# dmalyuta/explicit_hybrid_mpc

Hardware: AMD Instinct MI355X
Metric: oracle LP solves/sec + final regions/sec, 4-state 2-input N=5 hybrid MPC (higher is better)
Workload: dtype f64

## Files before the change

explicit_hybrid_mpc_amd/_capi.py:

```python

import ctypes
import os
import numpy as np

from . import build as _build

c_double_p = ctypes.POINTER(ctypes.c_double)
c_int32_p = ctypes.POINTER(ctypes.c_int32)
c_uint8_p = ctypes.POINTER(ctypes.c_uint8)

EHM_OK = 0
EHM_E_INVALID = -1
EHM_E_NO_DEVICE = -2
EHM_E_HIP = -3
EHM_E_CAPACITY = -4
EHM_E_INFEASIBLE = -5
EHM_E_NUMERIC = -6
PERSIST_FAMILIES = ('none', 'k2', 'kp', 'kpm', 'k4')
EHM_MAX_P = 8

EXPORTED = [
    'ehm_problem_create', 'ehm_problem_destroy', 'ehm_problem_set_eps', 'ehm_sync',
    'ehm_stream', 'ehm_solve_ptd_batch', 'ehm_feas_ptd_batch', 'ehm_solve_pt_batch',
    'ehm_vr_batch', 'ehm_slack_batch', 'ehm_bar_e_batch', 'ehm_min_simplex_batch',
# ... 64 lines not shown


class NodeInit(ctypes.Structure):
    _fields_ = [('delta', c_uint8_p), ('vcost', c_double_p), ('vinput', c_double_p)]


class TreeInfo(ctypes.Structure):
    _fields_ = [('n_nodes', ctypes.c_int64), ('n_leaves', ctypes.c_int64),
                ('n_roots', ctypes.c_int64), ('n_closed', ctypes.c_int64),
                ('lp_solves', ctypes.c_int64), ('ref_solves', ctypes.c_int64),
                ('ipm_iters', ctypes.c_int64), ('sweeps', ctypes.c_int64),
                ('max_depth', ctypes.c_int32), ('truncated', ctypes.c_int32),
                ('volume_closed', ctypes.c_double), ('min_margin', ctypes.c_double),
                ('device_seconds', ctypes.c_double), ('decide_seconds', ctypes.c_double),
                ('expand_seconds', ctypes.c_double), ('decide_launches', ctypes.c_int64),
                ('expand_launches', ctypes.c_int64), ('decide_solves', ctypes.c_int64),
                ('decide_iters', ctypes.c_int64), ('replicated_closed', ctypes.c_int64),
                ('replicated_nodes', ctypes.c_int64), ('replicated_solves', ctypes.c_int64),
                ('cert_closed', ctypes.c_int64), ('witness_open', ctypes.c_int64),
                ('swaps', ctypes.c_int64), ('blacklisted', ctypes.c_int64),
                ('kind_solves', ctypes.c_int64 * 5), ('kind_iters', ctypes.c_int64 * 5),
                ('near_threshold', ctypes.c_int64), ('witness_inherited', ctypes.c_int64),
                ('midpoints_shared', ctypes.c_int64),
                ('persist_ticks', ctypes.c_int64 * 10), ('witness_table', ctypes.c_int64)]


class Progress(ctypes.Structure):
    _fields_ = [('n_nodes', ctypes.c_int64), ('n_closed', ctypes.c_int64),
                ('frontier', ctypes.c_int64), ('sweeps', ctypes.c_int64),
                ('lp_solves', ctypes.c_int64), ('ipm_iters', ctypes.c_int64),
                ('depth', ctypes.c_int32), ('reserved', ctypes.c_int32),
                ('volume_closed', ctypes.c_double), ('n_splits', ctypes.c_int64)]


class PwaLaw(ctypes.Structure):
    _fields_ = [('n_x', ctypes.c_int32), ('n_u', ctypes.c_int32), ('n_modes', ctypes.c_int32),
                ('N', ctypes.c_int32), ('A', c_double_p), ('B', c_double_p), ('w', c_double_p),
                ('region_rows', c_int32_p), ('Hx', c_double_p), ('hx', c_double_p),
                ('n_gx', ctypes.c_int32), ('Gx', c_double_p), ('gx', c_double_p),
                ('n_gu', ctypes.c_int32), ('Gu', c_double_p), ('gu', c_double_p),
                ('n_q', ctypes.c_int32), ('Q', c_double_p),
                ('n_r', ctypes.c_int32), ('R', c_double_p)]


POINTS_FN = ctypes.CFUNCTYPE(ctypes.c_int, ctypes.c_void_p, ctypes.c_int64, ctypes.c_void_p,
                             ctypes.c_void_p, ctypes.c_int32, ctypes.c_int32, ctypes.c_void_p,
                             ctypes.c_void_p)
# ... 235 lines not shown
```

explicit_hybrid_mpc_amd/csrc/ehm_capi.hip:

```cpp
#include <hip/hip_runtime.h>

#include <algorithm>
#include <cmath>
#include <cstdarg>
#include <cstdio>
#include <cstdlib>
#include <cstring>
#include <memory>
#include <set>
#include <string>
#include <vector>

#include "../../include/ehmpc.h"
#include "ehm_host.h"

#define EHM_MAX_P_DEV 8
#include "ehm_kernels.h"
#include "ehm_k2.h"
#include "ehm_implicit.h"

using namespace ehm;

#define EHM_K2_NPS(X, S) X(8, S) X(12, S) X(16, S) X(20, S) X(24, S) X(28, S) X(32, S)
#define EHM_K2_ALL(X) EHM_K2_NPS(X, 1) EHM_K2_NPS(X, 2) EHM_K2_NPS(X, 3) EHM_K2_NPS(X, 4)
// ... 403 lines not shown
    DevBuf rec, left, didx, depth, flags, tstar, grad, wit, mt_state, mt_data;
};

struct ehm_problem {
    int device = 0;
    Stream stream;
    DevProblem dp{};
    int delta_len = 0;
    std::vector<uint8_t> deltas;
    DevBuf consts;
    DevBuf wc2;
    DevBuf wc4;
    DevBuf wr3;
    DevBuf quad;
    bool quadratic = false;
    bool k2q_ok = false;
    bool v1_ok = false;
    int decide_full = 0;
    int mid_first = 1;
    int inherit_wit = 1;
    bool budget_keep = false;
    bool check_witness = false;
    int work_first = 1;
    int share_mid = 1;
    int any_admissible = 0;
    int hy_timing = 0;
    int solver_gen = 2;
    DevBuf seg;
    std::set<const K2Api*> k2_ready;
    std::set<const KpApi*> kp_ready;
    NodePool pool_cache;
    DevBuf fr_a, fr_b, open_flag, open_list, d_count;
    DevBuf pq_slots, pq_ctl;
    DevBuf in0, in1, in2, out0, out1, out2, out3;
    DevBuf ex_stage, ex_tmp;
    DevBuf d_cnt;
    DevCounters* counters() const { return d_cnt.as<DevCounters>(); }
    struct ehm_tree* active_run = nullptr;
    std::vector<struct ehm_tree*> trees;
    Event bev[2];
    double batch_seconds[2] = {0.0, 0.0};
    long long batch_launches[2] = {0, 0};
    long long launches = 0;
    long long fallbacks = 0;
    long long slivers = 0;
    int num_cu = 256;
// ... 6 lines not shown
    ehm_problem* prob = nullptr;
    int device = 0;
    std::unique_ptr<HyState> hy;
    DevTree dt{};
    NodePool pool;
    long long limit = 0;
    DevBuf code;
    ehm_tree_info info{};
    int skip_volume = 0;
    int32_t persist_kernel[4] = {0, 0, 0, 0};
    bool unordered = false;
    bool keep_ids = false;
    DevBuf d_perm, d_inv;
    bool have_perm = false;
    struct Run {
        bool active = false;
        int max_depth = 0, action = 0, shard_world = 1, shard_rank = 0, engine = 0;
        int deal_depth = 0;
        long long shard_min = 0;
        bool sharded = true, cur_is_a = true;
        long long n_roots = 0, n_nodes = 0, nf = 0, n_closed = 0, ref_solves = 0;
        long long pre_closed = 0, pre_nodes = 0, pre_solves = 0, given = 0, received = 0;
        long long pre_first = 0;
        int sweeps = 0, depth = 0, truncated = 0;
        DevCounters c0{};
        Event ev0;
        std::vector<Event> evs;
        std::vector<int> ev_kind;
    } run;
    ~ehm_tree();
};

static int map_deltas(ehm_problem* P, int64_t n_inst, const uint8_t* delta,
                      std::vector<int32_t>& out) {
    out.resize((size_t)n_inst);
    const int L = P->delta_len;
    for (int64_t k = 0; k < n_inst; ++k) {
        int found = -1;
        if (!delta) {
            found = 0;
        } else {
            for (int d = 0; d < P->dp.n_delta; ++d) {
                bool eq = true;
                for (int q = 0; q < L && eq; ++q)
                    eq = ((delta[k * L + q] != 0) == (P->deltas[(size_t)d * L + q] != 0));
                if (eq) {
// ... 510 lines not shown
    if (!strcmp(name, "solver")) return ehm_problem_set_solver(P, (int)value);
    if (!strcmp(name, "decide_full")) {
        P->decide_full = value != 0.0;
        return EHM_OK;
    }
    if (!strcmp(name, "timing")) {
        P->hy_timing = value != 0.0;
        return EHM_OK;
    }
    if (!strcmp(name, "mid_first")) {
        P->mid_first = value != 0.0;
        return EHM_OK;
    }
    if (!strcmp(name, "inherit_witness")) {
        P->inherit_wit = value != 0.0;
        return EHM_OK;
    }
    if (!strcmp(name, "work_first")) {
        P->work_first = value != 0.0;
        return EHM_OK;
    }
    if (!strcmp(name, "check_witness")) {
        P->check_witness = value != 0.0;
        return EHM_OK;
    }
    if (!strcmp(name, "budget_keep")) {
        P->budget_keep = value != 0.0;
        return EHM_OK;
    }
    if (!strcmp(name, "share_midpoints")) {
        P->share_mid = value != 0.0;
        return EHM_OK;
    }
    if (!strcmp(name, "any_admissible")) {
        if (value < 0.0 || value > 2e9) return fail(EHM_E_INVALID, "any_admissible: seed + 1, or 0");
        if (P->active_run)
            return fail(EHM_E_INVALID, "any_admissible: not while a partition run is active");
        P->any_admissible = (int)value;
        return EHM_OK;
    }
    return fail(EHM_E_INVALID, "unknown option '%s'", name);
}

int ehm_sync(ehm_problem* P) {
    if (!P) return fail(EHM_E_INVALID, "null problem");
    HIP_TRY(hipStreamSynchronize(P->stream), EHM_E_HIP);
// ... 1302 lines not shown
                }
                const size_t lds = (shared + (size_t)nw * wave) * sizeof(double);
                const long long reg_wg = (kp->max_threads / 64) / nw;
                const long long wg_per_cu =
                    std::max<long long>(1, std::min<long long>(EHM_LDS_BUDGET / lds, reg_wg));
                cfg.L.grid = (int)((long long)P->num_cu * wg_per_cu);
                cfg.L.threads = (int)(64 * nw);
                cfg.L.lds_bytes = lds;
                cfg.L.wave_doubles = (int)wave;
            }
        }
    }
    const long long waves = (long long)cfg.L.grid * (cfg.L.threads / 64);
    const long long n_slots = 2 * T->limit + waves + 64;
    if (n_slots > 0x7fffffffLL || T->limit >= (long long)EHM_REQUEUED)
        return fail(EHM_E_INVALID, "node pool too large for the persistent engine");
    HIP_TRY(P->pq_slots.ensure((size_t)n_slots * 4), EHM_E_HIP);
    HIP_TRY(P->pq_ctl.ensure(sizeof(PersistCtl)), EHM_E_HIP);
    int32_t* slots = P->pq_slots.as<int32_t>();
    HIP_TRY(hipMemsetAsync(slots, 0xFF, (size_t)n_slots * 4, P->stream), EHM_E_HIP);
    const int32_t* cur = (R.cur_is_a ? P->fr_a : P->fr_b).as<int32_t>();
    HIP_TRY(hipMemcpyAsync(slots, cur, (size_t)R.nf * 4, hipMemcpyDeviceToDevice, P->stream),
            EHM_E_HIP);
    PersistDeal deal{0, 0, 0, 1, 0, 0};
    deal.check = P->check_witness ? 1 : 0;
    T->dt.code = nullptr;
    if (dealt) {
        deal = PersistDeal{0, R.deal_depth, R.shard_rank, R.shard_world,
                           getenv("EHM_DEAL_LOW_BITS") ? 0 : 1, 0, P->check_witness ? 1 : 0};
        HIP_TRY(T->code.ensure((size_t)T->pool.cap * 4), EHM_E_HIP);
        T->dt.code = T->code.as<uint32_t>();
        std::vector<uint32_t> codes((size_t)R.n_roots);
        for (long long k = 0; k < R.n_roots; ++k) codes[(size_t)k] = (uint32_t)k;
        HIP_TRY(hipMemcpyAsync(T->dt.code, codes.data(), codes.size() * 4, hipMemcpyHostToDevice,
                               P->stream), EHM_E_HIP);
        HIP_TRY(hipStreamSynchronize(P->stream), EHM_E_HIP);
    }
    if (max_pops > 0 && max_pops < n_slots) deal.pop_limit = (int)max_pops;
    deal.keep = (P->work_first && !getenv("EHM_NO_WORKFIRST")) ? 1 : 0;
    if (deal.pop_limit > 0 && !P->budget_keep) deal.keep = 0;
    PersistCtl h{};
    h.head = 0;
    h.tail = (int)R.nf;
    h.pending = (int)R.nf;
    h.n_nodes = (int)R.n_nodes;
    HIP_TRY(hipMemcpyAsync(P->pq_ctl.ptr, &h, sizeof h, hipMemcpyHostToDevice, P->stream),
            EHM_E_HIP);
    R.evs.push_back(Event::recorded(P->stream));
    if (kp) {
        T->persist_kernel[0] = kp_mid ? EHM_PERSIST_KPM : EHM_PERSIST_KP;
        T->persist_kernel[1] = kp->np_decide;
        T->persist_kernel[2] = kp->np_expand;
        T->persist_kernel[3] = kp->slots;
    } else {
        T->persist_kernel[0] = cfg.api == ehm_k4_api() ? EHM_PERSIST_K4 : EHM_PERSIST_K2;
        T->persist_kernel[1] = cfg.api->np;
        T->persist_kernel[2] = cfg.api->np;
        T->persist_kernel[3] = cfg.api->slots;
    }
    (kp ? kp->persist : cfg.api->persist)(cfg.L, P->dp, T->dt, slots, (int)n_slots,
                                          P->pq_ctl.as<PersistCtl>(), (int)T->limit, P->counters(),
                                          P->decide_full ? 0 : 1, R.max_depth, deal);
    R.evs.push_back(Event::recorded(P->stream));
    R.ev_kind.push_back(0);
    P->launches++;
    HIP_TRY(hipGetLastError(), EHM_E_HIP);
    HIP_TRY(hipMemcpyAsync(&h, P->pq_ctl.ptr, sizeof h, hipMemcpyDeviceToHost, P->stream),
            EHM_E_HIP);
    HIP_TRY(hipStreamSynchronize(P->stream), EHM_E_HIP);
    if (h.abort == 1)
        return fail(EHM_E_CAPACITY, "node pool exhausted at %d nodes (max_nodes=%lld)",
                    h.n_nodes, T->limit);
    const long long left_over =
        (deal.pop_limit > 0 && h.tail > deal.pop_limit) ? (long long)h.tail - deal.pop_limit : 0;
    if (h.abort != 0 || h.pending != left_over)
        return fail(EHM_E_HIP, "persistent frontier kernel stopped early (abort=%d, pending=%d, "
                               "expected %lld)", h.abort, h.pending, left_over);
    if (left_over > 0) {
        DevBuf& fb = P->fr_a;
        HIP_TRY(fb.ensure((size_t)left_over * 4 * 2), EHM_E_HIP);
        HIP_TRY(hipMemcpyAsync(fb.ptr, slots + deal.pop_limit, (size_t)left_over * 4,
                               hipMemcpyDeviceToDevice, P->stream), EHM_E_HIP);
        HIP_TRY(hipStreamSynchronize(P->stream), EHM_E_HIP);
        R.cur_is_a = true;
    }
    R.ref_solves += (long long)h.closed + 3LL * (long long)h.splits;
    if (deal.world > 1) {
        R.pre_closed = (long long)h.repl_closed;
        R.pre_nodes = R.n_roots + 2LL * (long long)h.repl_splits;
        R.pre_solves = (long long)h.repl_solves;
        R.sharded = true;
    }
    R.n_closed += (long long)h.closed;
    R.n_nodes = h.n_nodes;
    R.truncated = R.truncated || h.truncated;
    R.depth = std::max(R.depth, h.max_depth_seen);
    R.sweeps = R.depth + 1;
    R.nf = left_over;
    T->unordered = true;
    return EHM_OK;
}

int ehm_partition_advance(ehm_tree* T, int64_t max_pops, int64_t* frontier_size) {
    if (!T || !T->run.active) return fail(EHM_E_INVALID, "no partition run in progress");
    ehm_problem* P = T->prob;
    auto& R = T->run;
    if (T->hy || P->solver_gen != 2 || P->dp.Wr3)
        return fail(EHM_E_INVALID, "ehm_partition_advance: needs a single-commutation problem on "
                                   "the shared-block kernels (use ehm_partition_step)");
// ... 337 lines not shown
    T->info.n_nodes = R.n_nodes;
    T->info.n_roots = R.n_roots;
    T->info.n_leaves = R.n_nodes - (R.n_nodes - R.n_roots - received) / 2;
    T->info.n_closed = R.n_closed;
    T->info.lp_solves = (int64_t)(c1.lp_solves - R.c0.lp_solves);
    T->info.ipm_iters = (int64_t)(c1.ipm_iters - R.c0.ipm_iters);
    T->info.ref_solves = R.ref_solves;
    T->info.sweeps = R.sweeps;
    T->info.max_depth = R.depth;
    T->info.truncated = R.truncated;
    T->info.device_seconds = ms * 1e-3;
    T->info.decide_seconds = t_kind[0];
    T->info.expand_seconds = t_kind[1];
    T->info.decide_launches = n_kind[0];
    T->info.expand_launches = n_kind[1];
    T->info.decide_solves = (int64_t)(c1.slack_solves - R.c0.slack_solves);
    T->info.decide_iters = (int64_t)(c1.slack_iters - R.c0.slack_iters);
    T->info.cert_closed = (int64_t)(c1.cert_closed - R.c0.cert_closed);
    T->info.witness_open = (int64_t)(c1.wit_open - R.c0.wit_open);
    T->info.witness_inherited = (int64_t)(c1.wit_inherited - R.c0.wit_inherited);
    T->info.midpoints_shared = (int64_t)(c1.mid_shared - R.c0.mid_shared);
    T->info.witness_table = (int64_t)(c1.wit_table - R.c0.wit_table);
    for (int k = 0; k < 10; ++k) T->info.persist_ticks[k] = (int64_t)(c1.prof[k] - R.c0.prof[k]);
    T->info.near_threshold = (int64_t)(c1.routed - R.c0.routed);
    T->info.replicated_closed = R.pre_closed;
    T->info.replicated_nodes = R.pre_nodes;
    T->info.replicated_solves = R.pre_solves;
    {
        double mm;
        std::memcpy(&mm, &c1.min_margin_bits, 8);
        T->info.min_margin = mm;
    }
    for (int k = 0; k < 5; ++k) T->info.kind_solves[k] = T->info.kind_iters[k] = 0;
    T->info.kind_solves[LP_SLACK] = T->info.decide_solves;
    T->info.kind_iters[LP_SLACK] = T->info.decide_iters;
    T->info.kind_solves[LP_POINT] = T->info.lp_solves - T->info.decide_solves;
    T->info.kind_iters[LP_POINT] = T->info.ipm_iters - T->info.decide_iters;
    T->info.swaps = 0;
    T->info.blacklisted = 0;
    if (T->hy) {
        rc = hy_kind_totals(T, T->info.kind_solves, T->info.kind_iters);
        if (rc) return rc;
        T->info.decide_solves = T->info.kind_solves[LP_MIN_SIMPLEX] + T->info.kind_solves[LP_SLACK] +
                                T->info.kind_solves[LP_FEAS_SIMPLEX];
        T->info.decide_iters = T->info.kind_iters[LP_MIN_SIMPLEX] + T->info.kind_iters[LP_SLACK] +
                               T->info.kind_iters[LP_FEAS_SIMPLEX];
// ... 152 lines not shown
```

explicit_hybrid_mpc_amd/csrc/ehm_k2.h:

```cpp
#pragma once

#include <hip/hip_runtime.h>
#include <stdint.h>

#include "ehm_dev.h"

#ifndef EHM_K2_THREADS
#define EHM_K2_THREADS 768
#endif

#define K2_AUG_MIN 32
#define K2_HOT_GRAD 176
#define EHM_ROUTE_TOL 1e-6
#define EHM_REQUEUED 0x40000000

namespace ehm {

__host__ __device__ inline size_t k2_node_doubles(int p, int n_u) {
    const size_t nrec = ((size_t)rec_doubles(p, n_u) + 7) & ~(size_t)7;
    const size_t aug = (2 * (size_t)p * p > K2_AUG_MIN) ? 2 * (size_t)p * p : K2_AUG_MIN;
    return (nrec + aug + (size_t)p * p + 8 + 1) & ~(size_t)1;
}

__host__ __device__ inline int k2_stash_doubles(int p, int n_u) {
// ... 5 lines not shown
    const int r = m & 63;
    return (r != 0 && r + ne <= 64) ? m : ((m + 63) & ~63);
}
__host__ __device__ inline int lp_slots(int m, int ne) {
    return (lp_xbase(m, ne) + ne + 63) >> 6;
}

struct PersistCtl {
    int head;
    int pad0[31];
    int tail;
    int pad1[31];
    int pending;
    int pad2[31];
    int n_nodes;
    int pad3[31];
    int abort;
    int max_depth_seen;
    int truncated;
    int pad4;
    unsigned long long closed;
    unsigned long long splits;
    unsigned long long repl_closed, repl_splits, repl_solves;
};

struct PersistDeal {
    int pop_limit;
    int depth, rank, world;
    int mix;
    int keep;
    int check;
};

struct K2Gather {
    const long long* src;
    const int32_t* dst;
    const int32_t* n_dev;
    int v_off;
    double* grad;
    int sign_mode;
    MidTable pt;
};

struct K2Launch {
    int grid;
    int threads;
    size_t lds_bytes;
    int wave_doubles;
    hipStream_t stream;
    int wc_lds;
};

struct K2Api {
    int np, slots, max_threads, threads_per_lp;
// ... 34 lines not shown
```

explicit_hybrid_mpc_amd/csrc/ehm_persist.h:

```cpp
#ifndef EHM_PERSIST_H
#define EHM_PERSIST_H

#ifndef kx_persist
#error "kx_persist (the kernel's name) must be defined, and the namespace aliases kd / ke declared"
#endif

#define EHM_PERSIST_WATCHDOG_TICKS (60LL * 100000000LL)
#ifndef EHM_PERSIST_MIDFIRST
#define EHM_PERSIST_MIDFIRST 0
#endif
__global__ __launch_bounds__(EHM_K2_THREADS) void kx_persist(
    DevProblem P, DevTree T, int32_t* slots, int n_slots, PersistCtl* ctl, int node_cap,
    DevCounters* cnt, int wave_doubles, int sign_only, int max_depth, PersistDeal deal) {
    double* sm = reinterpret_cast<double*>(k2_smem);
    const int tid = threadIdx.x;
    const int lane0 = tid & 63;
    const int wave = __builtin_amdgcn_readfirstlane(tid >> 6);
    kd::Shared S;
    kd::carve_shared(S, sm, P);
    ke::Shared Se;
    ke::carve_shared(Se, sm, P);
#if EHM2_PROF
    S.gprof = cnt ? cnt->phase : nullptr;
    Se.gprof = cnt ? cnt->phase : nullptr;
#endif
    kd::NodeBuf nb;
    kd::carve_node(nb, sm + kd::shared_doubles(P) + (size_t)wave * wave_doubles, P.p, P.n_u);
    ke::NodeBuf nbe;
    ke::carve_node(nbe, sm + kd::shared_doubles(P) + (size_t)wave * wave_doubles, P.p, P.n_u);
    const int p = P.p, n_u = P.n_u;
    const int nrec = rec_doubles(p, n_u);
    kd::load_shared(P, 0, sm, tid, blockDim.x);
    __syncthreads();
    const long long t_start = wall_clock64();
    unsigned long long* wst = reinterpret_cast<unsigned long long*>(nb.aug);
    double* wmargin = nb.aug + 16;
    enum { W_SOLVES = 0, W_ITERS, W_STALLED, W_ERRORS, W_SLACK, W_SLACK_ITERS, W_CLOSED, W_SPLITS,
           W_DEPTH, W_TRUNC, W_CERT, W_WIT, W_ROUTED, W_RCLOSED, W_RSPLITS, W_RSOLVES,
           W_INH = 17, W_MT = 18, W_MTPARK = 19,
           W_TQ = 20, W_TMT = 21, W_TMID = 22, W_TSLK = 23, W_NMT = 24,
           W_WITT = 25, W_TPRE = 26, W_TPOST = 27, W_REQ = 28 };
    if (lane0 < 29 && lane0 != 16) wst[lane0] = 0ULL;
    if (lane0 == 0) *wmargin = 1e300;
    kd::wsync();
    int keep = -1;
    bool hot = false;
    int hot_dep = 0, hot_d = 0;
    const bool keep_child = deal.keep != 0;
    for (;;) {
        int id = -1;
        const bool is_hot = hot && keep >= 0;
        hot = false;
        if (keep >= 0) {
            id = keep;
            keep = -1;
        } else if (lane0 == 0) {
            const int idx = atomicAdd(&ctl->head, 1);
            if (idx < ((deal.pop_limit > 0 && deal.pop_limit < n_slots) ? deal.pop_limit
                                                                        : n_slots)) {
                long long t_q = 0;
                for (;;) {
                    id = __hip_atomic_load(&slots[idx], __ATOMIC_RELAXED, __HIP_MEMORY_SCOPE_AGENT);
                    if (id >= 0) break;
                    if (!t_q) t_q = wall_clock64();
                    if (__hip_atomic_load(&ctl->pending, __ATOMIC_RELAXED,
                                          __HIP_MEMORY_SCOPE_AGENT) <= 0 ||
                        __hip_atomic_load(&ctl->abort, __ATOMIC_RELAXED,
                                          __HIP_MEMORY_SCOPE_AGENT) != 0)
                        break;
                    if (wall_clock64() - t_start > EHM_PERSIST_WATCHDOG_TICKS) {
// ... 15 lines not shown
        double* hgrad = nb.lp + K2_HOT_GRAD;
        const int ng = (p + 1) * p;
        int dep = hot_dep;
        if (!is_hot) {
            __builtin_amdgcn_fence(__ATOMIC_ACQUIRE, "agent");
            const double* rec = T.rec + (size_t)id * T.rec_stride;
            const double g_in = (T.grad && lane < ng) ? T.grad[(size_t)id * ng + lane] : 0.0;
#if EHM_PERSIST_MIDFIRST
            const double w_in = (T.wit && sign_only && lane < p + 2)
                ? T.wit[(size_t)id * (p + 2) + lane] : 0.0;
#endif
            dep = T.depth[id];
            for (int k = lane; k < nrec; k += 64) node[k] = rec[k];
            if (T.grad) {
                if (lane < ng) hgrad[lane] = g_in;
                for (int k = lane + 64; k < ng; k += 64) hgrad[k] = T.grad[(size_t)id * ng + k];
            }
#if EHM_PERSIST_MIDFIRST
            if (T.wit && sign_only && lane < p + 2)
                nb.rec[(size_t)wave_doubles - k2_stash_doubles(p, n_u) + n_u + p + lane] = w_in;
#endif
        }
        kd::wsync();
        bool inh_open = false;
        double inh_tw = 0.0;
#if EHM_PERSIST_MIDFIRST
        if (T.wit && sign_only) {
            const double* wit_ = nb.rec + (size_t)wave_doubles - k2_stash_doubles(p, n_u) + n_u + p;
            const double* Vc = node + rec_off_vcost(p);
            double vbw = 0.0;
            for (int q = 0; q <= p; ++q) vbw = fma(wit_[1 + q], Vc[q], vbw);
            const double cw = wit_[0];
            const double tw = fmin(vbw - cw - P.eps_a, vbw - (1.0 + P.eps_r) * cw);
            inh_open = tw > EHM_ROUTE_TOL * (1.0 + fabs(vbw));
            inh_tw = tw;
        }
#endif
        if (T.grad && sign_only && inh_open && deal.check) {
            const double thr = -EHM_ROUTE_TOL * (1.0 + fabs(node[rec_off_vcost(p)]));
            const double bnd = cut_bound(node, hgrad, p, P.eps_a, P.eps_r, lane, nb.lp, thr);
            if (bnd < thr && lane == 0) wst[W_ERRORS] += 1;
            kd::wsync();
        }
        if (T.grad && sign_only && !inh_open) {
            const double thr = -EHM_ROUTE_TOL * (1.0 + fabs(node[rec_off_vcost(p)]));
            const double bnd = cut_bound(node, hgrad, p, P.eps_a, P.eps_r, lane, nb.lp, thr);
            if (bnd < thr) {
                if (lane == 0) {
                    const int dep0 = dep;
                    wst[W_CERT] += 1;
                    wst[W_CLOSED] += 1;
                    if (dep0 < deal.depth) wst[W_RCLOSED] += 1;
                    *wmargin = fmin(*wmargin, -bnd);
                    if ((unsigned long long)dep0 > wst[W_DEPTH]) wst[W_DEPTH] = (unsigned long long)dep0;
                    T.tstar[id] = bnd;
                    if (is_hot) T.flags[id] = 3;
                    else T.flags[id] |= 1;
                    atomicSub(&ctl->pending, 1);
                }
                kd::wsync();
                continue;
            }
        }
#if EHM_PERSIST_MIDFIRST
        const bool can_split = !(max_depth > 0 && dep >= max_depth);
        double* mid = nb.th;
        const int st_g = n_u, st_w = n_u + p;
        double* stash = nb.rec + (size_t)wave_doubles - k2_stash_doubles(p, n_u);
        double* wit = stash + st_w;
        bool have_wit = false;
        int mt_res = MT_NONE;
        int bi = 0, bj = 1;
        int its = 0;
        double Jm = 0.0;
        int mid_status = 1, mid_iters = 0;
        bool mid_conv = false;
        bool open = false;
        double tst = 0.0, margin = 0.0;
        bool decided = false;
        if (T.wit && sign_only) {
            if (inh_open) {
                open = true;
                decided = true;
                have_wit = true;
                tst = inh_tw;
                margin = inh_tw;
                if (lane == 0) wst[W_INH] += 1;
            }
        }
        if (can_split) {
            longest_edge_wave(node, p, lane, bi, bj);
            if (lane < p) {
#pragma clang fp contract(off)
                mid[lane] = (node[bi * p + lane] + node[bj * p + lane]) / 2.0;
            }
            kd::wsync();
            if (T.mt.state) {
                unsigned int mt_i = 0u;
                int mt_slot = 0;
                const unsigned long long mt_tg = mt_tag(mid, p, T.mt.mask, &mt_i);
                if (lane == 0) {
                    wst[W_TPRE] += (unsigned long long)(wall_clock64() - t_pre);
// ... 4 lines not shown
                                      &mt_slot, &waited, may_requeue);
                    if (mt_res == MT_BUSY) {
                        const int t = atomicAdd(&ctl->tail, 1);
                        if (t < n_slots) {
                            __hip_atomic_store(&slots[t], id | EHM_REQUEUED, __ATOMIC_RELAXED,
                                               __HIP_MEMORY_SCOPE_AGENT);
                            wst[W_REQ] += 1;
                        } else {
                            mt_res = mt_claim(T.mt, mt_tg, mt_i, t_start,
                                              EHM_PERSIST_WATCHDOG_TICKS, &mt_slot, &waited);
                        }
                    }
                    if (waited) {
                        wst[W_TMT] += (unsigned long long)waited;
                        wst[W_NMT] += 1;
                    }
                }
                mt_res = __builtin_amdgcn_readfirstlane(mt_res);
                mt_slot = __builtin_amdgcn_readfirstlane(mt_slot);
                if (mt_res == MT_BUSY) {
                    kd::wsync();
                    continue;
                }
                if (mt_res == MT_HIT) {
                    bool same = false;
                    const double ev = mt_read(T.mt, mt_slot, lane, mid, p, &same);
                    if (!same) {
                        mt_res = MT_NONE;
                    } else {
                        const int word = (int)__shfl(ev, 9);
                        Jm = __shfl(ev, 8);
                        mid_status = word & 0xff;
                        mid_conv = ((word >> 8) & 1) != 0;
                        mid_iters = 0;
                        if (lane >= 10 && lane < 10 + n_u) stash[lane - 10] = ev;
                        if (T.grad && lane >= 18 && lane < 18 + p) stash[st_g + lane - 18] = ev;
                        if (lane == 0) wst[W_MT] += 1;
                    }
                }
                if (lane == 0) wst[W_MTPARK] = (unsigned long long)mt_res |
                                               ((unsigned long long)mt_slot << 2);
            }
            if (mt_res != MT_HIT)
            {
            const long long t_mid = wall_clock64();
            ke::Wave Wm;
            ke::IpmResult rm;
            for (int attempt = 0; attempt < EHM2_ATTEMPTS; ++attempt) {
                double b[ke::SLOTS];
                const int ln = kd::pin(lane);
                ke::assemble_point(Se, Wm, nbe.lp, mid, false, b, ln, P, 0);
                rm = ke::ipm_solve(Se, Wm, b, ln, false, ke::step_fraction(attempt),
                                   T.grad ? nb.F : nullptr);
                its += rm.iters;
                if (rm.status == 0) break;
            }
#if EHM2_QUAD
            if (T.grad) ke::quad_grad_add(Wm, P, 0, mid, nb.F, lane);
#endif
            Jm = rm.obj;
            mid_status = rm.status;
            mid_conv = (rm.status == 0) && (rm.merit <= 1.0);
            mid_iters = its;
            if (lane < n_u) stash[lane] = Wm.xb[lane];
// ... 147 lines not shown
            if (margin < EHM_ROUTE_TOL * (1.0 + fabs(node[rec_off_vcost(p)]))) wst[W_ROUTED] += 1;
            if ((unsigned long long)dep > wst[W_DEPTH]) wst[W_DEPTH] = (unsigned long long)dep;
            T.tstar[id] = tst;
            if (!open) {
                T.flags[id] |= 1;
                wst[W_CLOSED] += 1;
                if (dep < deal.depth) wst[W_RCLOSED] += 1;
            }
        }
        if (!open) {
            if (lane == 0) atomicSub(&ctl->pending, 1);
            kd::wsync();
            continue;
        }
        if (!can_split) {
            if (lane == 0) {
                wst[W_TRUNC] = 1;
                atomicSub(&ctl->pending, 1);
            }
            kd::wsync();
            continue;
        }
        const long long t_post = wall_clock64();
        const bool fast = keep_child && !(deal.world > 1 && dep + 1 == deal.depth);
        const double gv0 = (T.grad && lane < ng) ? T.grad[(size_t)id * ng + lane] : 0.0;
        const int d = is_hot ? hot_d : T.didx[id];
        int c0 = 0;
        if (lane == 0) c0 = atomicAdd(&ctl->n_nodes, 2);
        c0 = __builtin_amdgcn_readfirstlane(c0);
        if (c0 + 2 > node_cap) {
            if (lane == 0) {
                atomicMax(&ctl->abort, 1);
                atomicSub(&ctl->pending, 1);
            }
            break;
        }
        struct { double obj; } r = {Jm};
        if (T.grad) {
            const double* gp_ = T.grad + (size_t)id * ng;
            double* g0 = T.grad + (size_t)c0 * ng;
            for (int k = lane; k < ng; k += 64) {
                const double gv = (k < 64) ? gv0 : gp_[k];
                const double a0 = (k >= bi * p && k < bi * p + p) ? stash[st_g + k - bi * p] : gv;
                const double a1 = (k >= bj * p && k < bj * p + p) ? stash[st_g + k - bj * p] : gv;
                __hip_atomic_store(g0 + k, a0, __ATOMIC_RELAXED, __HIP_MEMORY_SCOPE_AGENT);
                __hip_atomic_store(g0 + ng + k, a1, __ATOMIC_RELAXED, __HIP_MEMORY_SCOPE_AGENT);
                if (fast) hgrad[k] = a1;
            }
        }
        if (T.wit && lane < p + 2) {
            double* w0 = T.wit + (size_t)c0 * (p + 2);
            double v0 = 0.0, v1 = 0.0;
            if (have_wit) {
                witness_for_children(wit, node + rec_off_vcost(p), bi, bj, lane, v0, v1);
            }
            __hip_atomic_store(w0 + lane, v0, __ATOMIC_RELAXED, __HIP_MEMORY_SCOPE_AGENT);
            __hip_atomic_store(w0 + (p + 2) + lane, v1, __ATOMIC_RELAXED, __HIP_MEMORY_SCOPE_AGENT);
            kd::wsync();
            if (fast) wit[lane] = v1;
        }
        if (lane == 0) {
            wst[W_SPLITS] += 1;
            if (dep < deal.depth) wst[W_RSPLITS] += 1;
        }
        const double* xmid = stash;
#else
        kd::IpmResult r;
        int its = 0;
        {
            kd::Wave W;
            for (int attempt = 0; attempt < EHM2_ATTEMPTS; ++attempt) {
                double b[kd::SLOTS];
                const int ln = kd::pin(lane);
                kd::assemble_simplex(S, W, nb, node, node + rec_off_vcost(p), SX_SLACK, P.eps_a,
                                     P.eps_r, b, ln, P, 0);
                r = kd::ipm_solve(S, W, b, ln, sign_only != 0, kd::step_fraction(attempt));
                its += r.iters;
                if (r.status == 0) break;
            }
        }
        r.iters = its;
        const double tst = -r.obj;
// ... 97 lines not shown
        }
        const long long t_post = wall_clock64();
        const double* xmid = W.xb;
#endif
        double* rec0 = T.rec + (size_t)c0 * T.rec_stride;
        double* rec1 = rec0 + T.rec_stride;
        const int ov = rec_off_vcost(p), ou = rec_off_vinput(p);
        for (int k = lane; k < nrec; k += 64) {
            double v0 = node[k], v1 = node[k];
            if (k < ov) {
                if (k >= bi * p && k < bi * p + p) v0 = mid[k - bi * p];
                if (k >= bj * p && k < bj * p + p) v1 = mid[k - bj * p];
            } else if (k < ou) {
                if (k - ov == bi) v0 = r.obj;
                if (k - ov == bj) v1 = r.obj;
            } else {
                const int q = k - ou;
                if (q >= bi * n_u && q < bi * n_u + n_u) v0 = xmid[q - bi * n_u];
                if (q >= bj * n_u && q < bj * n_u + n_u) v1 = xmid[q - bj * n_u];
            }
            __hip_atomic_store(rec0 + k, v0, __ATOMIC_RELAXED, __HIP_MEMORY_SCOPE_AGENT);
            __hip_atomic_store(rec1 + k, v1, __ATOMIC_RELAXED, __HIP_MEMORY_SCOPE_AGENT);
#if EHM_PERSIST_MIDFIRST
            if (fast) node[k] = v1;
#endif
        }
        int own0 = 1, own1 = 1;
        if (lane == 0) {
            T.left[id] = c0;
#define EHM_WT(ptr, val) __hip_atomic_store((ptr), (val), __ATOMIC_RELAXED, __HIP_MEMORY_SCOPE_AGENT)
            if (T.code) {
                const uint32_t pc = T.code[id];
                const uint32_t code0 = 2u * pc, code1 = 2u * pc + 1u;
                EHM_WT(&T.code[c0], code0);
                EHM_WT(&T.code[c0 + 1], code1);
                if (deal.world > 1 && dep + 1 == deal.depth) {
                    const uint32_t h0 = deal.mix ? ((code0 * 2654435761u) >> 12) : code0;
                    const uint32_t h1 = deal.mix ? ((code1 * 2654435761u) >> 12) : code1;
                    own0 = (int)(h0 % (uint32_t)deal.world) == deal.rank;
                    own1 = (int)(h1 % (uint32_t)deal.world) == deal.rank;
                }
            }
            EHM_WT(&T.left[c0], -1);
            EHM_WT(&T.left[c0 + 1], -1);
            EHM_WT(&T.didx[c0], d);
            EHM_WT(&T.didx[c0 + 1], d);
            EHM_WT(&T.depth[c0], dep + 1);
            EHM_WT(&T.depth[c0 + 1], dep + 1);
            EHM_WT(&T.flags[c0], (uint8_t)(own0 ? 2 : 6));
            EHM_WT(&T.flags[c0 + 1], (uint8_t)(own1 ? 2 : 6));
            EHM_WT(&T.tstar[c0], 0.0);
            EHM_WT(&T.tstar[c0 + 1], 0.0);
#undef EHM_WT
        }
        __builtin_amdgcn_fence(__ATOMIC_RELEASE, "workgroup");
        __builtin_amdgcn_s_waitcnt(0);
        int kept = -1;
        if (lane == 0) {
            const int nown = own0 + own1;
            int push0 = own0, push1 = own1;
            if (keep_child) {
                if (own1) { kept = c0 + 1; push1 = 0; }
                else if (own0) { kept = c0; push0 = 0; }
            }
            const int npush = push0 + push1;
            const int t = npush ? atomicAdd(&ctl->tail, npush) : 0;
            if (t + npush <= n_slots) {
                int at = t;
                if (push0)
                    __hip_atomic_store(&slots[at++], c0, __ATOMIC_RELAXED, __HIP_MEMORY_SCOPE_AGENT);
                if (push1)
                    __hip_atomic_store(&slots[at], c0 + 1, __ATOMIC_RELAXED,
                                       __HIP_MEMORY_SCOPE_AGENT);
                if (nown != 1) atomicAdd(&ctl->pending, nown - 1);
            } else {
                kept = -1;
                atomicMax(&ctl->abort, 1);
                atomicSub(&ctl->pending, 1);
            }
            wst[W_TPOST] += (unsigned long long)(wall_clock64() - t_post);
        }
        keep = __builtin_amdgcn_readfirstlane(kept);
#if EHM_PERSIST_MIDFIRST
        hot = fast && keep >= 0;
        hot_dep = dep + 1;
        hot_d = d;
#endif
        kd::wsync();
    }
    kd::wsync();
    if (lane0 == 0) {
        atomicAdd(&cnt->lp_solves, wst[W_SOLVES]);
        atomicAdd(&cnt->ipm_iters, wst[W_ITERS]);
        if (wst[W_STALLED]) atomicAdd(&cnt->stalled, wst[W_STALLED]);
        if (wst[W_ERRORS]) atomicAdd(&cnt->errors, wst[W_ERRORS]);
        atomicAdd(&cnt->slack_solves, wst[W_SLACK]);
        atomicAdd(&cnt->slack_iters, wst[W_SLACK_ITERS]);
        atomicMin(&cnt->min_margin_bits, (unsigned long long)__double_as_longlong(*wmargin));
        if (wst[W_CERT]) atomicAdd(&cnt->cert_closed, wst[W_CERT]);
        if (wst[W_WIT]) atomicAdd(&cnt->wit_open, wst[W_WIT]);
        if (wst[W_INH]) atomicAdd(&cnt->wit_inherited, wst[W_INH]);
        if (wst[W_MT]) atomicAdd(&cnt->mid_shared, wst[W_MT]);
        if (wst[W_WITT]) atomicAdd(&cnt->wit_table, wst[W_WITT]);
        atomicAdd(&cnt->prof[0], (unsigned long long)(wall_clock64() - t_start));
        if (wst[W_TQ]) atomicAdd(&cnt->prof[1], wst[W_TQ]);
        if (wst[W_TMT]) atomicAdd(&cnt->prof[2], wst[W_TMT]);
        if (wst[W_TMID]) atomicAdd(&cnt->prof[3], wst[W_TMID]);
        if (wst[W_TSLK]) atomicAdd(&cnt->prof[4], wst[W_TSLK]);
        if (wst[W_NMT]) atomicAdd(&cnt->prof[5], wst[W_NMT]);
        if (wst[W_TPRE]) atomicAdd(&cnt->prof[6], wst[W_TPRE]);
        if (wst[W_TPOST]) atomicAdd(&cnt->prof[7], wst[W_TPOST]);
        if (wst[W_REQ]) atomicAdd(&cnt->prof[8], wst[W_REQ]);
        if (wst[W_ROUTED]) atomicAdd(&cnt->routed, wst[W_ROUTED]);
        atomicAdd(&ctl->closed, wst[W_CLOSED]);
        atomicAdd(&ctl->splits, wst[W_SPLITS]);
        if (wst[W_RCLOSED]) atomicAdd(&ctl->repl_closed, wst[W_RCLOSED]);
        if (wst[W_RSPLITS]) atomicAdd(&ctl->repl_splits, wst[W_RSPLITS]);
        if (wst[W_RSOLVES]) atomicAdd(&ctl->repl_solves, wst[W_RSOLVES]);
        atomicMax(&ctl->max_depth_seen, (int)wst[W_DEPTH]);
        if (wst[W_TRUNC]) atomicMax(&ctl->truncated, 1);
    }
}

#undef kx_persist

#endif
```

include/ehmpc.h:

```cpp
#ifndef EHMPC_H
#define EHMPC_H

#include <stddef.h>
#include <stdint.h>

#ifdef __cplusplus
extern "C" {
#endif
#if defined(__GNUC__)
#pragma GCC visibility push(default)
#endif

#define EHM_OK              0
#define EHM_E_INVALID      -1
#define EHM_E_NO_DEVICE    -2
#define EHM_E_HIP          -3
#define EHM_E_CAPACITY     -4
#define EHM_E_INFEASIBLE   -5
#define EHM_E_NUMERIC      -6

#define EHM_MAX_N   64
#define EHM_MAX_M   1024
#define EHM_MAX_P   8

// ... 141 lines not shown
    double  volume_closed;
    double  min_margin;
    double  device_seconds;
    double  decide_seconds;
    double  expand_seconds;
    int64_t decide_launches;
    int64_t expand_launches;
    int64_t decide_solves;
    int64_t decide_iters;
    int64_t replicated_closed;
    int64_t replicated_nodes;
    int64_t replicated_solves;
    int64_t cert_closed;
    int64_t witness_open;
    int64_t swaps;
    int64_t blacklisted;
    int64_t kind_solves[5];
    int64_t kind_iters[5];
    int64_t near_threshold;
    int64_t witness_inherited;
    int64_t midpoints_shared;
    int64_t persist_ticks[10];
    int64_t witness_table;
} ehm_tree_info;

int ehm_tree_info_get(const ehm_tree* tree, ehm_tree_info* out);
int ehm_tree_export(const ehm_tree* tree, double* vertices, int32_t* left, int32_t* right,
                    int32_t* delta_idx, double* vcost, double* vinput, uint8_t* flags,
                    double* tstar);
int ehm_tree_destroy(ehm_tree* tree);
int ehm_host_alloc(size_t bytes, void** out);
int ehm_host_free(void* ptr);



typedef struct ehm_explicit ehm_explicit;
int ehm_explicit_create(int device, int64_t n_nodes, int32_t n_roots, int32_t p, int32_t n_u,
                        const int32_t* left, const int32_t* right, const double* vertices,
                        const double* vinput, ehm_explicit** out);
int ehm_explicit_eval_batch(ehm_explicit* ex, int64_t n, const double* x, double* u,
                            int32_t* leaf, int32_t* visited, double* kernel_seconds);
int ehm_explicit_destroy(ehm_explicit* ex);
const char* ehm_explicit_last_error(void);

typedef struct ehm_compiled ehm_compiled;
int ehm_compiled_create(ehm_explicit* src, const double* vertices, ehm_compiled** out,
// ... 113 lines not shown
```

Measured before the change: 9.882 million.

## Eagerly certify children with LP-free bounds before pushing to persistent queue

After splitting a node, the persistent kernel now runs the LP-free witness/cut-bound verdict on both children right away and marks certified ones closed instead of pushing them onto the work queue. It also allocates child node slots earlier once the decision is known, and stages the left child's record in wave scratch so either child can be kept hot. The intent is to cut queue traffic and pop/reload work for children that close trivially. The cost is extra bound evaluation per split plus a new counter for pushes, and scratch offsets in nb.lp are assumed to fit.

```diff
diff --git a/explicit_hybrid_mpc_amd/_capi.py b/explicit_hybrid_mpc_amd/_capi.py
--- a/explicit_hybrid_mpc_amd/_capi.py
+++ b/explicit_hybrid_mpc_amd/_capi.py
@@ -110,7 +110,8 @@
                 ('kind_solves', ctypes.c_int64 * 5), ('kind_iters', ctypes.c_int64 * 5),
                 ('near_threshold', ctypes.c_int64), ('witness_inherited', ctypes.c_int64),
                 ('midpoints_shared', ctypes.c_int64),
-                ('persist_ticks', ctypes.c_int64 * 10), ('witness_table', ctypes.c_int64)]
+                ('persist_ticks', ctypes.c_int64 * 10), ('witness_table', ctypes.c_int64),
+                ('persist_pushes', ctypes.c_int64)]
 
 
 class Progress(ctypes.Structure):
diff --git a/explicit_hybrid_mpc_amd/csrc/ehm_capi.hip b/explicit_hybrid_mpc_amd/csrc/ehm_capi.hip
--- a/explicit_hybrid_mpc_amd/csrc/ehm_capi.hip
+++ b/explicit_hybrid_mpc_amd/csrc/ehm_capi.hip
@@ -449,6 +449,7 @@
     bool budget_keep = false;
     bool check_witness = false;
     int work_first = 1;
+    int eager_children = 1;
     int share_mid = 1;
     int any_admissible = 0;
     int hy_timing = 0;
@@ -501,6 +502,7 @@
         long long n_roots = 0, n_nodes = 0, nf = 0, n_closed = 0, ref_solves = 0;
         long long pre_closed = 0, pre_nodes = 0, pre_solves = 0, given = 0, received = 0;
         long long pre_first = 0;
+        long long pushes = 0;
         int sweeps = 0, depth = 0, truncated = 0;
         DevCounters c0{};
         Event ev0;
@@ -1057,6 +1059,10 @@
     }
     if (!strcmp(name, "check_witness")) {
         P->check_witness = value != 0.0;
+        return EHM_OK;
+    }
+    if (!strcmp(name, "eager_children")) {
+        P->eager_children = value != 0.0;
         return EHM_OK;
     }
     if (!strcmp(name, "budget_keep")) {
@@ -2405,12 +2411,12 @@
     const int32_t* cur = (R.cur_is_a ? P->fr_a : P->fr_b).as<int32_t>();
     HIP_TRY(hipMemcpyAsync(slots, cur, (size_t)R.nf * 4, hipMemcpyDeviceToDevice, P->stream),
             EHM_E_HIP);
-    PersistDeal deal{0, 0, 0, 1, 0, 0};
+    PersistDeal deal{0, 0, 0, 1, 0, 0, 0, 0};
     deal.check = P->check_witness ? 1 : 0;
     T->dt.code = nullptr;
     if (dealt) {
         deal = PersistDeal{0, R.deal_depth, R.shard_rank, R.shard_world,
-                           getenv("EHM_DEAL_LOW_BITS") ? 0 : 1, 0, P->check_witness ? 1 : 0};
+                           getenv("EHM_DEAL_LOW_BITS") ? 0 : 1, 0, P->check_witness ? 1 : 0, 0};
         HIP_TRY(T->code.ensure((size_t)T->pool.cap * 4), EHM_E_HIP);
         T->dt.code = T->code.as<uint32_t>();
         std::vector<uint32_t> codes((size_t)R.n_roots);
@@ -2422,6 +2428,7 @@
     if (max_pops > 0 && max_pops < n_slots) deal.pop_limit = (int)max_pops;
     deal.keep = (P->work_first && !getenv("EHM_NO_WORKFIRST")) ? 1 : 0;
     if (deal.pop_limit > 0 && !P->budget_keep) deal.keep = 0;
+    deal.eager = P->eager_children ? 1 : 0;
     PersistCtl h{};
     h.head = 0;
     h.tail = (int)R.nf;
@@ -2468,6 +2475,7 @@
         R.cur_is_a = true;
     }
     R.ref_solves += (long long)h.closed + 3LL * (long long)h.splits;
+    R.pushes += (long long)h.pushes;
     if (deal.world > 1) {
         R.pre_closed = (long long)h.repl_closed;
         R.pre_nodes = R.n_roots + 2LL * (long long)h.repl_splits;
@@ -2851,6 +2859,7 @@
     T->info.midpoints_shared = (int64_t)(c1.mid_shared - R.c0.mid_shared);
     T->info.witness_table = (int64_t)(c1.wit_table - R.c0.wit_table);
     for (int k = 0; k < 10; ++k) T->info.persist_ticks[k] = (int64_t)(c1.prof[k] - R.c0.prof[k]);
+    T->info.persist_pushes = R.pushes;
     T->info.near_threshold = (int64_t)(c1.routed - R.c0.routed);
     T->info.replicated_closed = R.pre_closed;
     T->info.replicated_nodes = R.pre_nodes;
diff --git a/explicit_hybrid_mpc_amd/csrc/ehm_k2.h b/explicit_hybrid_mpc_amd/csrc/ehm_k2.h
--- a/explicit_hybrid_mpc_amd/csrc/ehm_k2.h
+++ b/explicit_hybrid_mpc_amd/csrc/ehm_k2.h
@@ -51,6 +51,7 @@
     unsigned long long closed;
     unsigned long long splits;
     unsigned long long repl_closed, repl_splits, repl_solves;
+    unsigned long long pushes;
 };
 
 struct PersistDeal {
@@ -59,6 +60,7 @@
     int mix;
     int keep;
     int check;
+    int eager;
 };
 
 struct K2Gather {
diff --git a/explicit_hybrid_mpc_amd/csrc/ehm_persist.h b/explicit_hybrid_mpc_amd/csrc/ehm_persist.h
--- a/explicit_hybrid_mpc_amd/csrc/ehm_persist.h
+++ b/explicit_hybrid_mpc_amd/csrc/ehm_persist.h
@@ -39,13 +39,15 @@
            W_DEPTH, W_TRUNC, W_CERT, W_WIT, W_ROUTED, W_RCLOSED, W_RSPLITS, W_RSOLVES,
            W_INH = 17, W_MT = 18, W_MTPARK = 19,
            W_TQ = 20, W_TMT = 21, W_TMID = 22, W_TSLK = 23, W_NMT = 24,
-           W_WITT = 25, W_TPRE = 26, W_TPOST = 27, W_REQ = 28 };
-    if (lane0 < 29 && lane0 != 16) wst[lane0] = 0ULL;
+           W_WITT = 25, W_TPRE = 26, W_TPOST = 27, W_REQ = 28,
+           W_EAGER = 29, W_PUSH = 30 };
+    if (lane0 < 31 && lane0 != 16) wst[lane0] = 0ULL;
     if (lane0 == 0) *wmargin = 1e300;
     kd::wsync();
     int keep = -1;
     bool hot = false;
     int hot_dep = 0, hot_d = 0;
+    bool hot_tested = false;
     const bool keep_child = deal.keep != 0;
     for (;;) {
         int id = -1;
@@ -107,20 +109,56 @@
 #endif
         }
         kd::wsync();
+#if EHM_PERSIST_MIDFIRST
+        auto lp_free_verdict = [&](const double* rec_, const double* g_, const double* w_,
+                                   bool bound_done, double& tw, double& bnd) -> int {
+            bool w_open = false;
+            if (T.wit && sign_only) {
+                const double* Vc = rec_ + rec_off_vcost(p);
+                double vbw = 0.0;
+                for (int q = 0; q <= p; ++q) vbw = fma(w_[1 + q], Vc[q], vbw);
+                const double cw = w_[0];
+                tw = fmin(vbw - cw - P.eps_a, vbw - (1.0 + P.eps_r) * cw);
+                w_open = tw > EHM_ROUTE_TOL * (1.0 + fabs(vbw));
+            }
+            if (!(T.grad && sign_only) || bound_done || (w_open && !deal.check)) return w_open ? 1 : 0;
+            const double thr = -EHM_ROUTE_TOL * (1.0 + fabs(rec_[rec_off_vcost(p)]));
+            bnd = cut_bound(rec_, g_, p, P.eps_a, P.eps_r, lane, nb.lp, thr);
+            if (w_open) {
+                if (bnd < thr && lane == 0) wst[W_ERRORS] += 1;
+                kd::wsync();
+                return 1;
+            }
+            return bnd < thr ? 2 : 0;
+        };
         bool inh_open = false;
         double inh_tw = 0.0;
-#if EHM_PERSIST_MIDFIRST
-        if (T.wit && sign_only) {
-            const double* wit_ = nb.rec + (size_t)wave_doubles - k2_stash_doubles(p, n_u) + n_u + p;
-            const double* Vc = node + rec_off_vcost(p);
-            double vbw = 0.0;
-            for (int q = 0; q <= p; ++q) vbw = fma(wit_[1 + q], Vc[q], vbw);
-            const double cw = wit_[0];
-            const double tw = fmin(vbw - cw - P.eps_a, vbw - (1.0 + P.eps_r) * cw);
-            inh_open = tw > EHM_ROUTE_TOL * (1.0 + fabs(vbw));
-            inh_tw = tw;
-        }
-#endif
+        {
+            double bnd = 0.0;
+            const int verdict = lp_free_verdict(
+                node, hgrad, nb.rec + (size_t)wave_doubles - k2_stash_doubles(p, n_u) + n_u + p,
+                is_hot && hot_tested, inh_tw, bnd);
+            inh_open = verdict == 1;
+            if (verdict == 2) {
+                if (lane == 0) {
+                    const int dep0 = dep;
+                    wst[W_CERT] += 1;
+                    wst[W_CLOSED] += 1;
+                    if (dep0 < deal.depth) wst[W_RCLOSED] += 1;
+                    *wmargin = fmin(*wmargin, -bnd);
+                    if ((unsigned long long)dep0 > wst[W_DEPTH]) wst[W_DEPTH] = (unsigned long long)dep0;
+                    T.tstar[id] = bnd;
+                    if (is_hot) T.flags[id] = 3;
+                    else T.flags[id] |= 1;
+                    atomicSub(&ctl->pending, 1);
+                }
+                kd::wsync();
+                continue;
+            }
+        }
+#else
+        bool inh_open = false;
+        double inh_tw = 0.0;
         if (T.grad && sign_only && inh_open && deal.check) {
             const double thr = -EHM_ROUTE_TOL * (1.0 + fabs(node[rec_off_vcost(p)]));
             const double bnd = cut_bound(node, hgrad, p, P.eps_a, P.eps_r, lane, nb.lp, thr);
@@ -147,6 +185,7 @@
                 continue;
             }
         }
+#endif
 #if EHM_PERSIST_MIDFIRST
         const bool can_split = !(max_depth > 0 && dep >= max_depth);
         double* mid = nb.th;
@@ -163,6 +202,8 @@
         bool open = false;
         double tst = 0.0, margin = 0.0;
         bool decided = false;
+        int c0_early = 0;
+        bool alloc_early = false;
         if (T.wit && sign_only) {
             if (inh_open) {
                 open = true;
@@ -213,6 +254,10 @@
                     kd::wsync();
                     continue;
                 }
+                if (deal.eager && decided) {
+                    alloc_early = true;
+                    if (lane == 0) c0_early = atomicAdd(&ctl->n_nodes, 2);
+                }
                 if (mt_res == MT_HIT) {
                     bool same = false;
                     const double ev = mt_read(T.mt, mt_slot, lane, mid, p, &same);
@@ -231,6 +276,9 @@
                 }
                 if (lane == 0) wst[W_MTPARK] = (unsigned long long)mt_res |
                                                ((unsigned long long)mt_slot << 2);
+            } else if (deal.eager && decided) {
+                alloc_early = true;
+                if (lane == 0) c0_early = atomicAdd(&ctl->n_nodes, 2);
             }
             if (mt_res != MT_HIT)
             {
@@ -424,11 +472,17 @@
             continue;
         }
         const long long t_post = wall_clock64();
-        const bool fast = keep_child && !(deal.world > 1 && dep + 1 == deal.depth);
+        const bool dealt = deal.world > 1 && dep + 1 == deal.depth;
+        const bool fast = keep_child && !dealt;
+        const bool eager = deal.eager != 0 && sign_only && T.grad && !dealt;
+        const bool stage = fast || eager;
+        double* hg0 = nb.lp + 256;
+        double* cw0 = nb.lp + 328;
+        double* c0rec = nb.lp + 340;
         const double gv0 = (T.grad && lane < ng) ? T.grad[(size_t)id * ng + lane] : 0.0;
         const int d = is_hot ? hot_d : T.didx[id];
-        int c0 = 0;
-        if (lane == 0) c0 = atomicAdd(&ctl->n_nodes, 2);
+        int c0 = c0_early;
+        if (!alloc_early && lane == 0) c0 = atomicAdd(&ctl->n_nodes, 2);
         c0 = __builtin_amdgcn_readfirstlane(c0);
         if (c0 + 2 > node_cap) {
             if (lane == 0) {
@@ -447,7 +501,8 @@
                 const double a1 = (k >= bj * p && k < bj * p + p) ? stash[st_g + k - bj * p] : gv;
                 __hip_atomic_store(g0 + k, a0, __ATOMIC_RELAXED, __HIP_MEMORY_SCOPE_AGENT);
                 __hip_atomic_store(g0 + ng + k, a1, __ATOMIC_RELAXED, __HIP_MEMORY_SCOPE_AGENT);
-                if (fast) hgrad[k] = a1;
+                if (stage) hgrad[k] = a1;
+                if (eager) hg0[k] = a0;
             }
         }
         if (T.wit && lane < p + 2) {
@@ -459,7 +514,8 @@
             __hip_atomic_store(w0 + lane, v0, __ATOMIC_RELAXED, __HIP_MEMORY_SCOPE_AGENT);
             __hip_atomic_store(w0 + (p + 2) + lane, v1, __ATOMIC_RELAXED, __HIP_MEMORY_SCOPE_AGENT);
             kd::wsync();
-            if (fast) wit[lane] = v1;
+            if (stage) wit[lane] = v1;
+            if (eager) cw0[lane] = v0;
         }
         if (lane == 0) {
             wst[W_SPLITS] += 1;
@@ -603,9 +659,37 @@
             __hip_atomic_store(rec0 + k, v0, __ATOMIC_RELAXED, __HIP_MEMORY_SCOPE_AGENT);
             __hip_atomic_store(rec1 + k, v1, __ATOMIC_RELAXED, __HIP_MEMORY_SCOPE_AGENT);
 #if EHM_PERSIST_MIDFIRST
-            if (fast) node[k] = v1;
-#endif
-        }
+            if (stage) node[k] = v1;
+            if (eager) c0rec[k] = v0;
+#endif
+        }
+        int closed0 = 0, closed1 = 0;
+        double cbnd0 = 0.0, cbnd1 = 0.0;
+#if EHM_PERSIST_MIDFIRST
+        if (eager) {
+            kd::wsync();
+#pragma nounroll
+            for (int c = 0; c < 2; ++c) {
+                double tw_c = 0.0, bnd_c = 0.0;
+                const int verdict = lp_free_verdict(c ? node : c0rec, c ? hgrad : hg0,
+                                                    c ? wit : cw0, false, tw_c, bnd_c);
+                if (verdict == 2) {
+                    if (lane == 0) {
+                        wst[W_CERT] += 1;
+                        wst[W_CLOSED] += 1;
+                        wst[W_EAGER] += 1;
+                        if (dep + 1 < deal.depth) wst[W_RCLOSED] += 1;
+                        *wmargin = fmin(*wmargin, -bnd_c);
+                        if ((unsigned long long)(dep + 1) > wst[W_DEPTH])
+                            wst[W_DEPTH] = (unsigned long long)(dep + 1);
+                    }
+                    if (c) { closed1 = 1; cbnd1 = bnd_c; }
+                    else { closed0 = 1; cbnd0 = bnd_c; }
+                }
+                kd::wsync();
+            }
+        }
+#endif
         int own0 = 1, own1 = 1;
         if (lane == 0) {
             T.left[id] = c0;
@@ -628,23 +712,25 @@
             EHM_WT(&T.didx[c0 + 1], d);
             EHM_WT(&T.depth[c0], dep + 1);
             EHM_WT(&T.depth[c0 + 1], dep + 1);
-            EHM_WT(&T.flags[c0], (uint8_t)(own0 ? 2 : 6));
-            EHM_WT(&T.flags[c0 + 1], (uint8_t)(own1 ? 2 : 6));
-            EHM_WT(&T.tstar[c0], 0.0);
-            EHM_WT(&T.tstar[c0 + 1], 0.0);
+            EHM_WT(&T.flags[c0], (uint8_t)(closed0 ? 3 : own0 ? 2 : 6));
+            EHM_WT(&T.flags[c0 + 1], (uint8_t)(closed1 ? 3 : own1 ? 2 : 6));
+            EHM_WT(&T.tstar[c0], cbnd0);
+            EHM_WT(&T.tstar[c0 + 1], cbnd1);
 #undef EHM_WT
         }
         __builtin_amdgcn_fence(__ATOMIC_RELEASE, "workgroup");
         __builtin_amdgcn_s_waitcnt(0);
         int kept = -1;
         if (lane == 0) {
-            const int nown = own0 + own1;
-            int push0 = own0, push1 = own1;
+            const int need0 = own0 && !closed0, need1 = own1 && !closed1;
+            const int nown = need0 + need1;
+            int push0 = need0, push1 = need1;
             if (keep_child) {
-                if (own1) { kept = c0 + 1; push1 = 0; }
-                else if (own0) { kept = c0; push0 = 0; }
+                if (need1) { kept = c0 + 1; push1 = 0; }
+                else if (need0) { kept = c0; push0 = 0; }
             }
             const int npush = push0 + push1;
+            wst[W_PUSH] += (unsigned long long)npush;
             const int t = npush ? atomicAdd(&ctl->tail, npush) : 0;
             if (t + npush <= n_slots) {
                 int at = t;
@@ -663,7 +749,13 @@
         }
         keep = __builtin_amdgcn_readfirstlane(kept);
 #if EHM_PERSIST_MIDFIRST
-        hot = fast && keep >= 0;
+        if (eager && keep == c0) {
+            for (int k = lane; k < nrec; k += 64) node[k] = c0rec[k];
+            for (int k = lane; k < ng; k += 64) hgrad[k] = hg0[k];
+            if (T.wit && lane < p + 2) wit[lane] = cw0[lane];
+        }
+        hot = stage && keep >= 0;
+        hot_tested = eager;
         hot_dep = dep + 1;
         hot_d = d;
 #endif
@@ -692,6 +784,8 @@
         if (wst[W_TPRE]) atomicAdd(&cnt->prof[6], wst[W_TPRE]);
         if (wst[W_TPOST]) atomicAdd(&cnt->prof[7], wst[W_TPOST]);
         if (wst[W_REQ]) atomicAdd(&cnt->prof[8], wst[W_REQ]);
+        if (wst[W_EAGER]) atomicAdd(&cnt->prof[9], wst[W_EAGER]);
+        if (wst[W_PUSH]) atomicAdd(&ctl->pushes, wst[W_PUSH]);
         if (wst[W_ROUTED]) atomicAdd(&cnt->routed, wst[W_ROUTED]);
         atomicAdd(&ctl->closed, wst[W_CLOSED]);
         atomicAdd(&ctl->splits, wst[W_SPLITS]);
diff --git a/include/ehmpc.h b/include/ehmpc.h
--- a/include/ehmpc.h
+++ b/include/ehmpc.h
@@ -187,6 +187,7 @@
     int64_t midpoints_shared;
     int64_t persist_ticks[10];
     int64_t witness_table;
+    int64_t persist_pushes;
 } ehm_tree_info;
 
 int ehm_tree_info_get(const ehm_tree* tree, ehm_tree_info* out);
```

After: 10.35 million, median of 6. 4.7% higher.
